# hitbc/panSVR

Hardware: AMD Instinct MI355X
Metric: signal reads realigned/sec (150 bp PE); bit-exact CIGAR vs CPU ref (higher is better)
Workload: dtype u8/int32 (2-bit k-mers, 8-bit DP deltas, 32-bit scores); 1 GPU; configs[1]: 1000000 synthetic 150 bp PE signal read pairs per GPU vs 10000-anchor SV reference (11.8 Mbp), `panSVR aln` hot path; pairs_per_gpu=1000000, engines_per_gpu=1, in_process_rebases=0, index_hbm_bytes=2713674320, index_distribution=every rank uploads its own copy from host memory

## Files before the change

pansvr_amd/csrc/aln_device.h:

```cpp
#pragma once
#include <stdint.h>
#include "../../include/psvr_engine.h"

#if defined(__HIPCC__)
#include <hip/hip_runtime.h>
#define PSVR_HD __host__ __device__ __forceinline__
#define PSVR_HDN __host__ __device__
#else
#define PSVR_HD inline
#define PSVR_HDN
#endif

namespace psvr {

static const int kLenKmer = 20, kSeedStep = 5, kUniPosNMax = 32;
static const int kMaxOut = 6;
static const int kMaxReadLen = 1600;
static const int kFwd = 1, kRev = 0;
static const int kSegMax = 160;
static const int kCigMax = 256;
static const int kMemSlot = 32;

struct SvDev { uint32_t chr_id; uint32_t st_pos; int32_t end_offset; int32_t pad; };

// ... 98 lines not shown
	DevIndex idx;
	psvr_aln_params_t par;
	int8_t mat[25];
	long long n_pairs;
	const char *bases; const long long *base_off; const psvr_ori_t *ori;
	int32_t lmax;
	int32_t wmax;
	const int32_t *grand; long long grand_n; long long grand_base;
	const int32_t *hrand[2]; long long hrand_n; long long hrand_base[2];
	long long n_slots;
	const int32_t *src;
	long long *poff;
	int32_t *rcnt;
	long long *hoff; int32_t *hcnt;
	const uint8_t *force;
	uint8_t *active; uint8_t *unmapped; uint8_t *is_str; uint8_t *has_n4;
	uint8_t *has_mem;
	int32_t *str_list; unsigned int *str_cnt;
	int32_t *read_l;
	uint8_t *bin;
	uint64_t *rb;
	uint8_t *seed_list;
	Strand *strand;
	ChainCand *ccand; int32_t *n_ccand;
	psvr_read_hdr_t *rh; psvr_pair_result_t *pres;
	psvr_cand_t *cand;
	Arena<VMem> mem; Arena<USeed> us; PathN *path;
	Arena<Seg> seg; Arena<DpDesc> dp; Arena<CandWork> cw; Arena<uint32_t> cig;
	const psvr_extz_t *dp_ez; const uint32_t *dp_cig;
	const uint8_t *tseq_in; int32_t *stale_open;
	int32_t *any_h;
	int32_t trace;
	int32_t *err;
	unsigned long long *stats;
};

enum { ST_PROBES = 0, ST_HITS, ST_SEEDS, ST_DP, ST_SIMPLE, ST_CELLS, ST_READS, ST_CAND, ST_N };

PSVR_HD void stat_add(const Ctx &c, int k, unsigned long long v)
{
	if (!c.stats) return;
#if defined(__HIP_DEVICE_COMPILE__)
	atomicAdd(c.stats + k, v);
#else
	c.stats[k] += v;
#endif
}

PSVR_HD long long src_read(const Ctx &c, long long read)
{
	return c.src ? (long long)c.src[read >> 1] * 2 + (read & 1) : read;
}

PSVR_HD uint64_t fnv1a(uint64_t h, uint64_t v)
{
	for (int i = 0; i < 8; ++i) { h ^= (v >> (8 * i)) & 0xff; h *= 1099511628211ULL; }
	return h;
}

PSVR_HD bool bucket_occupied(const DevIndex &ix, uint64_t h)
{
#ifdef PSVR_EMU_SPARSE_HASH
	(void)ix, (void)h;
	return true;
#else
	return !ix.occ || ((ix.occ[h >> 5] >> (h & 31)) & 1u);
// ... 1700 lines not shown
```

pansvr_amd/csrc/engine.hip:

```cpp
#include <hip/hip_runtime.h>
#include <algorithm>
#include <cstring>
#include <mutex>
#include <string>
#include <thread>
#include <vector>
#include "common.h"
#include "engine_core.h"
#include "bam_emit_hooks.h"
#include "fastq_parsed.h"
#include "host_io.h"
#include "index_build.h"
#include "ksw_device.h"
#include "ksw_launch.h"
#include "scan.h"

namespace psvr {

int dp_params(const psvr_ksw_params_t *par, int variant, DpParams *P);

static const int kBlock = 256;
static inline unsigned grid_for(long long n, int block = kBlock) { return (unsigned)((n + block - 1) / block); }

__device__ __forceinline__ long long pair_of(const int32_t *work, long long i) { return work ? (long long)work[i] : i; }
// ... 403 lines not shown
				if (old == km) { atomicAdd(&cnt[h], 1u); break; }
				h = (h + 1) & mask;
			}
		}
		distinct += __popcll(__ballot(fresh));
	}
	if (!((uint32_t)distinct < (uint32_t)kn - 15u)) { if (lane == 0) c.is_str[read] = 0; continue; }
	uint8_t *sl = (uint8_t *)(cnt + tsize);
	for (int i = lane; i < kn; i += 64) {
		const unsigned long long km = get_kmer((uint32_t)i, rb);
		unsigned h = (unsigned)((km * 0x9E3779B97F4A7C15ull) >> 40) & mask;
		while (key[h] != km) h = (h + 1) & mask;
		sl[i] = cnt[h] >= 4 ? 0 : 1;
	}
	if (lane == 0) {
		c.is_str[read] = 1;
		int bg = 0, ed = 0;
		for (int o = 0; o < kSeedStep; ++o) {
			bg += sl[o] == 0, ed += sl[L - kLenKmer - o] == 0;
			sl[o] += 2, sl[L - kLenKmer - o] += 4;
		}
		if (bg < kSeedStep && ed < kSeedStep) {
			int tot = 0;
			for (int o = 0; tot < kSeedStep && o < kn; ++o) {
				if (sl[o] > 0) continue;
				sl[o] += 8, tot++;
			}
		}
	}
	uint8_t *out = c.seed_list + read * (long long)c.lmax;
	for (int i = lane; i < kn; i += 64) out[i] = sl[i];
	}
}
__global__ __launch_bounds__(kBlock) __attribute__((amdgpu_waves_per_eu(8, 8))) void k_seed(Ctx c, const int32_t *work, long long n, int mate, int lds_pitch)
{
	extern __shared__ __align__(16) uint64_t seed_lds[];
	long long i = blockIdx.x * (long long)blockDim.x + threadIdx.x;
	if (i >= 2 * n) return;
	const long long rs = (pair_of(work, i >> 1) * 2 + mate) * 2 + (i & 1);
	if (lds_pitch) {
		uint64_t *mine = seed_lds + (size_t)threadIdx.x * lds_pitch;
		if (c.active[rs >> 1]) {
			const uint64_t *src = c.rb + rs * (long long)c.wmax;
			for (int k = 0; k < c.wmax; ++k) mine[k] = src[k];
		}
		seed_strand_t<true>(c, rs, mine);
	} else seed_strand_t<false>(c, rs, nullptr);
}
__global__ __launch_bounds__(kBlock) void k_scan_batch(const char *bases, const long long *off, const psvr_ori_t *ori, long long P, int match, int32_t *list, unsigned int *cnt_lmax)
{
	const long long p = blockIdx.x * (long long)blockDim.x + threadIdx.x;
	int lmax = 0, nn[2] = {0, 0};
	if (p < P) {
#pragma unroll
		for (int k = 0; k < 2; ++k) {
			const long long r = 2 * p + k, o = off[r], L = off[r + 1] - o;
			lmax = max(lmax, (int)(L < 0x7fffffff ? L : 0x7fffffff));
			const psvr_ori_t q = ori[r];
			const bool unm = q.unmapped || (uint32_t)q.chr_id > 24u;
			if ((!unm && q.align_score == (uint32_t)(L * match)) || L < kLenKmer || L > kMaxReadLen) continue;
			const uintptr_t a0 = (uintptr_t)(bases + o), a1 = a0 + (uintptr_t)L;
			int n = 0;
			for (uintptr_t a = a0 & ~(uintptr_t)3; a < a1; a += 4) {
				uint32_t x = *(const uint32_t *)a ^ 0x4E4E4E4Eu;
				if (a < a0) x |= 0xffffffffu >> (8 * (4 - (unsigned)(a0 - a)));
				if (a + 4 > a1) x |= 0xffffffffu << (8 * (unsigned)(a1 - a));
				const uint32_t z = ~(((x & 0x7F7F7F7Fu) + 0x7F7F7F7Fu) | x | 0x7F7F7F7Fu);
				n += __popc(z);
			}
			nn[k] = n < 255 ? n : 255;
		}
		if (nn[0] + nn[1] >= 1) {
// ... 14 lines not shown
	int32_t val[kListItems];
	unsigned int rank[kListItems];
	bool has[kListItems];
#pragma unroll
	for (int k = 0; k < kListItems; ++k) {
		const long long i = base + (long long)k * kBlock + threadIdx.x;
		has[k] = i < n_items && pred(i, val[k]);
		const unsigned long long m = __ballot(has[k]);
		unsigned int w0 = 0;
		if ((threadIdx.x & 63) == 0 && m) w0 = atomicAdd(&n_blk, (unsigned int)__popcll(m));
		rank[k] = (unsigned int)__builtin_amdgcn_readfirstlane((int)w0) + (unsigned int)__popcll(m & ((1ull << (threadIdx.x & 63)) - 1));
	}
	__syncthreads();
	if (threadIdx.x == 0 && n_blk) b_blk = atomicAdd(cnt, n_blk);
	__syncthreads();
#pragma unroll
	for (int k = 0; k < kListItems; ++k) if (has[k]) list[b_blk + rank[k]] = val[k];
}
__global__ __launch_bounds__(kBlock) void k_mem_list(Ctx c, const int32_t *work, long long n, int mate, int32_t *list, unsigned int *cnt)
{
	compact_list(n, list, cnt, [&](long long i, int32_t &read) {
		const long long r = pair_of(work, i) * 2 + mate;
		read = (int32_t)r;
		return c.active[r] && c.has_mem[r];
	});
}
__global__ __launch_bounds__(kBlock) void k_chain_small(Ctx c, const int32_t *list, const unsigned int *cnt)
{
	const long long i = blockIdx.x * (long long)blockDim.x + threadIdx.x;
	if (i >= (long long)*cnt) return;
	const int32_t r = list[i];
	if (chain_select_small(c, r)) return;
	chain_read(c, r), select_read(c, r);
}
__global__ __launch_bounds__(kBlock) void k_pair_dev(Ctx c, const int32_t *list, const unsigned long long *cnt)
{
	const unsigned long long n = *cnt;
	for (unsigned long long i = blockIdx.x * (unsigned long long)blockDim.x + threadIdx.x; i < n; i += (unsigned long long)gridDim.x * blockDim.x) pair_reads(c, list[i]);
}
__global__ __launch_bounds__(kBlock) void k_walk_list(Ctx c, const int32_t *work, long long n, int32_t *list, unsigned int *cnt)
{
	compact_list(2 * n, list, cnt, [&](long long i, int32_t &read) {
		const long long r = pair_of(work, i >> 1) * 2 + (i & 1);
		read = (int32_t)r;
		return c.active[r] && c.n_ccand[r] > 0;
	});
}
template <class T> __device__ __forceinline__ long long block_arena_alloc(const Arena<T> &a, unsigned long long n)
{
	__shared__ unsigned long long wsum[kBlock / 64];
	__shared__ long long bbase;
	const int lane = threadIdx.x & 63, wave = threadIdx.x >> 6, nw = (int)(blockDim.x >> 6);
	unsigned long long x = n;
#pragma unroll
	for (int o = 1; o < 64; o <<= 1) {
		const unsigned long long y = __shfl_up(x, o);
		if (lane >= o) x += y;
	}
	if (lane == 63) wsum[wave] = x;
	__syncthreads();
	if (threadIdx.x == 0) {
		unsigned long long tot = 0;
		for (int w = 0; w < nw; ++w) { const unsigned long long t = wsum[w]; wsum[w] = tot; tot += t; }
		long long b = 0;
		if (tot) {
			const unsigned long long o = atomicAdd(a.top, tot);
// ... 633 lines not shown
	}
	void unstage(Readbacks rb)
	{
		size_t at = 0;
		for (const Readback &x : rb) if (x.n) memcpy(x.h, (char *)pin + at, x.n), at += x.n;
	}
	hipEvent_t ev_early = nullptr;
	bool late_pending = false;
	int32_t *d2h_early_late(Readbacks early, const void *dl, size_t nl)
	{
		if (!ev_early && hipEventCreateWithFlags(&ev_early, hipEventDisableTiming) != hipSuccess) { d2h(early); return nullptr; }
		bool ok = true;
		const bool staged = queue_d2h(early, kLateAt, ok);
		note(hipEventRecord(ev_early, stream));
		const bool fits = staged && nl <= kPin - 4096 - kLateAt;
		if (fits) { note(hipMemcpyAsync((char *)pin + kLateAt, dl, nl, hipMemcpyDeviceToHost, stream)); late_pending = true; }
		note(hipEventSynchronize(ev_early));
		if (staged) unstage(early);
		return fits ? (int32_t *)((char *)pin + kLateAt) : nullptr;
	}
	void d2h_late_done() { if (late_pending) { note(hipStreamSynchronize(stream)); synced(); late_pending = false; } }
	~GpuBE()
	{
		if (pin) (void)hipHostFree(pin);
		if (up_ring) (void)hipHostFree(up_ring);
		if (ev_early) (void)hipEventDestroy(ev_early);
		if (ev_plan) (void)hipEventDestroy(ev_plan);
		for (int i = 0; i < kSide; ++i) {
			stream_pool().put(device, side[i]);
			if (ev_join[i]) (void)hipEventDestroy(ev_join[i]);
		}
		if (ev_fork) (void)hipEventDestroy(ev_fork);
	}
	void st_seed(const Ctx &c, const int32_t *w, long long n, int mate)
	{
		if (n > 0) {
			int pitch = c.wmax | 1;
			if ((size_t)pitch * 8 * kBlock > 64 * 1024) pitch = 0;
			t0("k_seed");
			hipLaunchKernelGGL(k_seed, dim3(grid_for(2 * n)), dim3(kBlock), (size_t)pitch * 8 * kBlock, stream, c, w, n, mate, pitch);
			t1();
			note(mem_list.ensure((size_t)(n + 4) * 4));
			note(hipMemsetAsync(mem_list.p, 0, 4, stream));
			hipLaunchKernelGGL(k_mem_list, dim3(grid_for(n, kBlock * kListItems)), dim3(kBlock), 0, stream, c, w, n, mate, mem_list.as<int32_t>() + 4, (unsigned int *)mem_list.p);
		}
		note(hipGetLastError());
	}
	DevBuf mem_list;
	void st_chain(const Ctx &c, const int32_t *w, long long n, int mate)
	{
		(void)w, (void)mate;
		if (n <= 0) return;
		t0("k_chain_small");
		hipLaunchKernelGGL(k_chain_small, dim3(grid_for(n)), dim3(kBlock), 0, stream, c, (const int32_t *)(mem_list.as<int32_t>() + 4), (const unsigned int *)mem_list.p);
		t1();
		note(hipGetLastError());
	}
	void st_pair_dev(const Ctx &c, const int32_t *list, const unsigned long long *cnt)
	{
		const long long blocks = c.n_pairs / kBlock + 1;
		hipLaunchKernelGGL(k_pair_dev, dim3((unsigned)(blocks < 2048 ? blocks : 2048)), dim3(kBlock), 0, stream, c, list, cnt);
		note(hipGetLastError());
	}
	static int str_tsize(const Ctx &c)
	{
		int tsize = 256;
		while (tsize < 2 * c.lmax) tsize <<= 1;
		return tsize;
	}
	DevBuf redo;
	static long long prep_pair_min() { static const long long v = [] { const char *e = getenv("PSVR_PREP_PAIR_MIN"); return e ? atoll(e) : 65536ll; }(); return v; }
	static int waves_for_lds(size_t per_wave, size_t fixed)
	{
		int w = kBlock / 64;
		while (w > 1 && fixed + (size_t)w * per_wave > (size_t)64 * 1024) w >>= 1;
		return w;
	}
	void launch_prep_wave(const Ctx &c, const int32_t *w, long long n, int mate, const unsigned int *n_dev, unsigned grid)
	{
		const int tsize = c.lmax <= 288 ? str_tsize(c) / 4 : str_tsize(c);
		const size_t per_wave = ((size_t)2 * c.lmax + (size_t)c.wmax * 8 + (size_t)tsize * 4 + 15) & ~(size_t)15;
		const int wpb = waves_for_lds(per_wave, 128);
		hipLaunchKernelGGL(k_prep, dim3(grid * (unsigned)(kBlock / 64 / wpb)), dim3(64 * wpb), (size_t)128 + (size_t)wpb * per_wave, stream, c, w, n, mate, tsize, (int)per_wave, n_dev);
	}
	void st_prep(const Ctx &c, const int32_t *w, long long n, int mate)
	{
		if (n <= 0) return;
		dzero(c.str_cnt, 4);
		if (c.lmax <= 288 && n >= prep_pair_min() && redo.ensure((size_t)(n + 4) * 4) == hipSuccess) {
			t0("k_prep");
			if (mate) {
				note(hipMemsetAsync(redo.p, 0, 4, stream));
				hipLaunchKernelGGL(k_prep_mate1, dim3(grid_for(n)), dim3(kBlock), 0, stream, c, w, n, redo.as<int32_t>() + 4, (unsigned int *)redo.p);
				launch_prep_wave(c, (const int32_t *)(redo.as<int32_t>() + 4), 0, 1, (const unsigned int *)redo.p, 64);
			} else if (c.lmax <= 160) hipLaunchKernelGGL((k_prep_pair<5, 256>), dim3(grid_for(n, 256)), dim3(256), (size_t)4 * 64 * (1 << (kPrepBits - 3)), stream, c, w, n, kPrepBits);
			else hipLaunchKernelGGL((k_prep_pair<9, 128>), dim3(grid_for(n, 128)), dim3(128), (size_t)2 * 64 * 512, stream, c, w, n, 12);
			t1();
			note(hipGetLastError());
			return;
		}
		t0("k_prep");
		launch_prep_wave(c, w, n, mate, nullptr, grid_for(n, kBlock / 64));
		t1();
		note(hipGetLastError());
	}
	void st_str(const Ctx &c, const int32_t *w, long long n, int mate)
	{
		if (n <= 0) return;
		const int tsize = str_tsize(c);
		const size_t per_wave = (size_t)tsize * 12 + (((size_t)c.lmax + 15) & ~(size_t)15);
		const int wpb = waves_for_lds(per_wave, 0);
		const size_t lds = (size_t)wpb * per_wave;
		t0("k_str_detect");
		const long long waves = n < 8192 ? n : 8192;
		hipLaunchKernelGGL(k_str_detect, dim3(grid_for(waves, wpb)), dim3(64 * wpb), lds, stream, c, w, n, mate, tsize, (int)per_wave);
		t1();
		note(hipGetLastError());
	}
#define PSVR_STAGE(name, kern, mult, blk)                                                                          \
	void name(const Ctx &c, const int32_t *w, long long n)                                                         \
	{                                                                                                              \
		if (n > 0) { t0(#kern); hipLaunchKernelGGL(kern, dim3(grid_for((mult) * n, blk)), dim3(blk), 0, stream, c, w, n); t1(); } \
		note(hipGetLastError());                                                                                   \
	}
	DevBuf walk_list;
	void st_walk(const Ctx &c, const int32_t *w, long long n)
	{
		if (n <= 0) return;
		note(walk_list.ensure((size_t)(2 * n + 4) * 4));
		int32_t *list = walk_list.as<int32_t>() + 4;
		unsigned int *cnt = (unsigned int *)walk_list.p;
		note(hipMemsetAsync(cnt, 0, 4, stream));
		hipLaunchKernelGGL(k_walk_list, dim3(grid_for(2 * n, kBlock * kListItems)), dim3(kBlock), 0, stream, c, w, n, list, cnt);
		t0("k_walk");
		hipLaunchKernelGGL(k_walk, dim3(grid_for(2 * n)), dim3(kBlock), 0, stream, c, (const int32_t *)list, (const unsigned int *)cnt);
		t1();
		note(hipGetLastError());
	}
	PSVR_STAGE(st_pair, k_pair, 1, kBlock)
	PSVR_STAGE(st_finalize_pair, k_finalize_pair, 1, kBlock)
#undef PSVR_STAGE
	DevBuf tmp_idx, tmp_val, tmp_out;
	void run_init(const RunInit &r)
	{
		long long n = r.S;
		for (long long k : {r.nsp, (long long)r.n_tops, (long long)r.n_atops, 16ll}) if (k > n) n = k;
		hipLaunchKernelGGL(k_run_init, dim3(grid_for(n)), dim3(kBlock), 0, stream, r);
		note(hipGetLastError());
	}
	void append_iota(int32_t *w, long long at, long long start, long long n) { if (n) hipLaunchKernelGGL(k_iota, dim3(grid_for(n)), dim3(kBlock), 0, stream, w, at, start, n); }
	void append_list(int32_t *w, long long at, const int32_t *src, long long n) { if (n) hipLaunchKernelGGL(k_copy_i32, dim3(grid_for(n)), dim3(kBlock), 0, stream, w, at, src, n); }
	void gather_listed(const long long *a, const long long *b, const int32_t *cc, const int32_t *idx, long long n, long long *oa, long long *ob, int32_t *oc)
	{
		if (!n) return;
		note(tmp_idx.ensure(n * 4)), note(tmp_out.ensure(n * 20 + 16));
		h2d(tmp_idx.p, idx, n * 4);
		hipLaunchKernelGGL(k_gather_listed, dim3(grid_for(n)), dim3(kBlock), 0, stream, a, b, cc, (const int32_t *)tmp_idx.p, n, (long long *)tmp_out.p);
		const char *o = (const char *)tmp_out.p;
		d2h({{oa, o, (size_t)n * 8}, {ob, o + n * 8, (size_t)n * 8}, {oc, o + n * 16, (size_t)n * 4}});
	}
	void scatter_listed_i32(int32_t *a, const int32_t *val, long long n)
	{
		if (!n) return;
		note(tmp_val.ensure(n * 4));
		h2d(tmp_val.p, val, n * 4);
// ... 644 lines not shown
{
	if (psvr_device_count() <= 0) return set_error(PSVR_ERR_DEVICE, "no HIP device visible: the engine has no CPU path");
	if (!e || !fq || !fq->valid || first_pair < 0 || n_pairs < 0 || first_pair + n_pairs > fq->last.n_pairs) return set_error(PSVR_ERR_ARG, "psvr_engine_upload_fastq: bad argument");
	if (fq->device != e->ix->device)
		return set_error(PSVR_ERR_ARG, "psvr_engine_upload_fastq: the text was parsed on device %d, the engine runs on device %d (the bases would have to travel between them)", fq->device, e->ix->device);
	PSVR_HIP(hipSetDevice(e->ix->device));
	e->be.stream = e->own;
	if (!e->committed) { e->core.commit(); e->committed = true; }
	e->compact_valid = false;
	e->src_fq = nullptr, e->ran = false;
	const int64_t *off = fq->base_off.as<int64_t>() + 2 * first_pair;
	long long b0 = 0, b1 = fq->last.total_bases;
	const bool whole = first_pair == 0 && n_pairs == fq->last.n_pairs;
	if (!whole && n_pairs > 0 && !e->be.d2h({{&b0, off, 8}, {&b1, off + 2 * n_pairs, 8}})) return engine_status(e, PSVR_ERR_DEVICE);
	const int rc = e->core.upload_device(n_pairs, fq->bases.as<char>(), off, fq->ori.as<psvr_ori_t>() + 2 * first_pair, b0, b1 - b0);
	const int st = engine_status(e, rc);
	if (!st) e->src_fq = fq, e->src_first = first_pair, e->src_n = n_pairs, e->src_generation = fq->generation;
	return st;
}

extern "C" int psvr_engine_run(psvr_engine_t *e, int trace, void *stream)
{
	if (!e) return set_error(PSVR_ERR_ARG, "psvr_engine_run: null engine");
	PSVR_HIP(hipSetDevice(e->ix->device));
	e->be.stream = stream ? (hipStream_t)stream : e->own;
	e->be.timing = (trace & 4) != 0;
	e->be.timed.clear();
	e->compact_valid = false;
	int rc = e->core.run(trace & 1, (trace & 2) != 0);
	hipError_t s = hipStreamSynchronize(e->be.stream);
	if (s != hipSuccess) e->be.note(s);
	e->be.synced();
	e->be.collect_timing();
	e->committed = false;
	const int st = engine_status(e, rc);
	e->ran = st == PSVR_OK;
	return st;
}

extern "C" int psvr_engine_set_stream_pos(psvr_engine_t *e, const int64_t pos[3])
{
	if (!e || !pos) return set_error(PSVR_ERR_ARG, "psvr_engine_set_stream_pos: null argument");
	PSVR_HIP(hipSetDevice(e->ix->device));
	e->core.have_run = false, e->committed = true;
	e->core.grand_pos = pos[0], e->core.hrand_pos[0] = pos[1], e->core.hrand_pos[1] = pos[2];
	return PSVR_OK;
}

extern "C" int psvr_engine_stream_end(psvr_engine_t *e, int64_t end[3])
{
	if (!e || !end) return set_error(PSVR_ERR_ARG, "psvr_engine_stream_end: null argument");
	PSVR_HIP(hipSetDevice(e->ix->device));
	long long t[3];
	e->core.stream_end(t);
	end[0] = t[0], end[1] = t[1], end[2] = t[2];
	return engine_status(e, PSVR_OK);
}

extern "C" int psvr_engine_rebase(psvr_engine_t *e, const int64_t pos[3], void *stream)
{
	if (!e || !pos) return set_error(PSVR_ERR_ARG, "psvr_engine_rebase: null argument");
	PSVR_HIP(hipSetDevice(e->ix->device));
	e->be.stream = stream ? (hipStream_t)stream : e->own;
	e->compact_valid = false;
	int rc = e->core.rebase(pos[0], pos[1], pos[2], e->core.c.trace, false);
	hipError_t s = hipStreamSynchronize(e->be.stream);
// ... 76 lines not shown
{
	std::lock_guard<std::mutex> lk(ix->emit_mu);
	if (!ix->emit_ready) {
		int cur = -1;
		(void)hipGetDevice(&cur);
		struct Back { int d; ~Back() { if (d >= 0) (void)hipSetDevice(d); } } back{cur};
		PSVR_HIP(hipSetDevice(ix->device));
		BeTableHost h;
		h.build((int)ix->host.svh.size(), [&](int i) { return ix->host.svh[(size_t)i].vcf_print_string.c_str(); }, [&](int i) { return ix->host.svh[(size_t)i].vcf_id.c_str(); });
		PSVR_HIP(ix->emit_text.alloc(h.text.size())); PSVR_HIP(ix->emit_off.alloc(h.off.size() * 4)); PSVR_HIP(ix->emit_tab.alloc(h.tab.size()));
		PSVR_HIP(hipMemcpy(ix->emit_text.p, h.text.data(), h.text.size(), hipMemcpyHostToDevice));
		PSVR_HIP(hipMemcpy(ix->emit_off.p, h.off.data(), h.off.size() * 4, hipMemcpyHostToDevice));
		PSVR_HIP(hipMemcpy(ix->emit_tab.p, h.tab.data(), h.tab.size(), hipMemcpyHostToDevice));
		ix->emit_ready = true;
	}
	T->text = ix->emit_text.as<char>(), T->off = ix->emit_off.as<uint32_t>(), T->tab = ix->emit_tab.as<uint8_t>();
	T->n_anchor = (int32_t)ix->host.svh.size(), T->n_header = ix->host.n_header;
	*device = ix->device;
	return PSVR_OK;
}
void psvr::engine_emit_view(const psvr_engine *e, EngineEmitView *v)
{
	const Ctx &c = e->core.c;
	v->device = e->ix->device, v->ran = e->ran && e->core.P > 0;
	v->fq = e->src_fq, v->first_pair = e->src_first, v->n_pairs = e->src_n, v->generation = e->src_generation;
	v->hdr = c.rh, v->pairs = c.pres, v->cands = c.cand, v->n_cands = (int64_t)c.cw.cap, v->cig = c.cig.base, v->n_cig = (int64_t)c.cig.cap;
}

extern "C" int psvr_engine_stats(const psvr_engine_t *e, char *buf, size_t n)
{
	if (!e || !buf || !n) return set_error(PSVR_ERR_ARG, "psvr_engine_stats: bad argument");
	const RunStats &s = e->core.stats;
	snprintf(buf, n,
	         "{\"pairs\":%lld,\"rounds\":%lld,\"pair_runs\":%lld,\"pair_only_runs\":%lld,\"shadow_runs\":%lld,\"sensitive_pairs\":%lld,\"window_misses\":%lld,\"adopted_pairs\":%lld,\"stale_open\":%lld,\"dp_problems\":%lld,\"dp_seq_bytes\":%lld,\"candidates\":%lld,\"walk_pairs\":%lld,\"walk_us\":%lld,\"n_special\":%lld,\"special_const\":%lld,\"special_nomove\":%lld,"
	         "\"probes\":%llu,\"hits\":%llu,\"seeds\":%llu,\"dp_cells\":%llu,\"simple\":%llu,\"reads_aligned\":%llu}",
	         e->core.P, s.rounds, s.pairs_run, s.pair_only, s.shadow_runs, s.sensitive, s.window_miss, s.adopted, s.stale_open, s.dp_problems, s.dp_seq_bytes, s.cands, s.walk_pairs, s.walk_us, s.n_special, s.special_const, s.special_nomove, s.counters[ST_PROBES], s.counters[ST_HITS], s.counters[ST_SEEDS],
	         s.counters[ST_CELLS], s.counters[ST_SIMPLE], s.counters[ST_READS]);
	std::string t = buf;
	t.pop_back();
	{
		size_t fr = 0, tot = 0;
		char b[96];
		if (hipSetDevice(e->ix->device) == hipSuccess && hipMemGetInfo(&fr, &tot) == hipSuccess) { snprintf(b, sizeof b, ",\"hbm_used_bytes\":%zu", tot - fr); t += b; }
	}
	t += ",\"kernels\":{";
	bool first = true;
	for (auto &k : e->be.timed) {
		char b[256];
		snprintf(b, sizeof b, "%s\"%s\":{\"ms\":%.4f,\"launches\":%lld}", first ? "" : ",", k.first.c_str(), k.second.first, k.second.second);
		t += b, first = false;
	}
	t += "}}";
	snprintf(buf, n, "%s", t.c_str());
	return PSVR_OK;
}
```

pansvr_amd/csrc/engine_core.h:

```cpp
#pragma once
#include <stdint.h>
#include <stdio.h>
#include <string.h>
#include <algorithm>
#include <atomic>
#include <cstdlib>
#include <initializer_list>
#include <mutex>
#include <string>
#include <thread>
#include <chrono>
#include <type_traits>
#include <vector>
#include "aln_device.h"
#include "dp_plan.h"

namespace psvr {

struct HostRand3 {
	int32_t ring[31];
	int f, b;
	void seed(unsigned s)
	{
		int32_t word = s ? (int32_t)s : 1;
// ... 41 lines not shown
		want = (want + 0xfffff) & ~0xfffffll;
		for (; k < want; ++k) {
			int32_t *&b = blk[k >> kLog];
			if (!b) b = new int32_t[(size_t)1 << kLog];
			b[k & kMask] = gen.next();
		}
		n.store(k, std::memory_order_release);
	}
	int32_t at(long long k) const { return blk[k >> kLog][k & kMask]; }
	void prefetch(long long k) const { if (k >= 0 && k < n.load(std::memory_order_relaxed)) __builtin_prefetch(blk[k >> kLog] + (k & kMask)); }
	template <class F> void pieces(long long from, long long cnt, F &&put) const
	{
		for (long long o = 0; o < cnt;) {
			const long long k = from + o, room = (kMask + 1) - (k & kMask), m = cnt - o < room ? cnt - o : room;
			put(o, blk[k >> kLog] + (k & kMask), m);
			o += m;
		}
	}
};
inline SharedRand &shared_grand() { static SharedRand s; return s; }

struct DpIO {
	long long begin, end;
	int32_t *qlen, *tlen;
	long long *q_off, *t_off;
	uint8_t *qbuf, *tbuf;
	psvr_extz_t *ez;
	uint32_t *cig;
	long long qbytes, tbytes, cig_words;
};

template <class B, class = void> struct plans_on_device : std::false_type {};
template <class B> struct plans_on_device<B, std::void_t<decltype(B::kDevicePlan)>> : std::true_type {};

struct Readback { void *h; const void *d; size_t n; };
typedef std::initializer_list<Readback> Readbacks;

struct HostMem {
	struct Buf {
		void *p = nullptr;
		size_t bytes = 0;
		Buf() = default;
		Buf(const Buf &) = delete;
		Buf &operator=(const Buf &) = delete;
		~Buf() { release(); }
		void release() { free(p); p = nullptr; bytes = 0; }
		bool alloc(size_t n)
		{
			release();
			p = calloc(n ? n : 1, 1);
			bytes = p ? n : 0;
			return p != nullptr;
		}
	};
	bool note(bool ok) { return ok; }
	void d2h(Readbacks rb) { for (const Readback &x : rb) if (x.n) memcpy(x.h, x.d, x.n); }
	void d2h(void *h, const void *d, size_t n) { d2h({{h, d, n}}); }
	std::vector<int32_t> late_buf;
	int32_t *d2h_early_late(Readbacks early, const void *dl, size_t nl)
	{
		d2h(early);
		late_buf.resize(nl / 4 + 1);
		memcpy(late_buf.data(), dl, nl);
		return late_buf.data();
	}
	void d2h_late_done() {}
	std::vector<int32_t> listed_idx;
	void gather_listed(const long long *a, const long long *b, const int32_t *cc, const int32_t *idx, long long n, long long *oa, long long *ob, int32_t *oc)
	{
		if (!n) return;
		listed_idx.assign(idx, idx + n);
		for (long long i = 0; i < n; ++i) oa[i] = a[idx[i]], ob[i] = b[idx[i]], oc[i] = cc[idx[i]];
	}
	void scatter_listed_i32(int32_t *a, const int32_t *val, long long n) { for (long long i = 0; i < n; ++i) a[listed_idx[i]] = val[i]; }
};

struct RunStats {
	long long rounds = 0, pairs_run = 0, pair_only = 0, shadow_runs = 0, sensitive = 0, window_miss = 0, dp_problems = 0, cands = 0, adopted = 0, stale_open = 0, dp_seq_bytes = 0, from_walk = 0;
	long long walk_pairs = 0, walk_us = 0, n_special = 0, special_const = 0, special_nomove = 0;
	unsigned long long counters[16] = {0};
};

template <class BE, class Mem = HostMem> struct EngineCore {
	BE &be;
	HostMem host;
	Mem &mem;
	typedef typename Mem::Buf Buf;
	template <class T> struct Dev : Buf { operator T *() const { return (T *)this->p; } };
	bool alloc_ok = true;
	template <class T> T *get(Dev<T> &b, unsigned long long n) { alloc_ok &= mem.note(b.alloc((n ? n : 1) * sizeof(T))); return b; }
	Ctx c;
	long long P = 0, R = 0;
	long long total_bases = 0;
	SharedRand &grand = shared_grand();
	RandStream hrand[2];
	long long grand_pos = 0, hrand_pos[2] = {0, 0};
	long long grand_dev_n = 0, hrand_dev_n = 0;
	long long grand_dev_base = 0, hrand_dev_base[2] = {0, 0}, grand_dev_cap = 0, hrand_dev_cap = 0;
	Dev<int32_t> d_grand, d_hrand[2];
	struct {
		Dev<long long> poff, hoff;
		Dev<int32_t> rcnt, hcnt, str_list, read_l, n_ccand;
		Dev<unsigned int> str_cnt;
		Dev<uint8_t> active, unmapped, is_str, has_n4, has_mem, bin, seed_list;
		Dev<uint64_t> rb;
		Dev<Strand> strand;
		Dev<ChainCand> ccand;
		Dev<psvr_read_hdr_t> rh;
		Dev<psvr_pair_result_t> pres;
		Dev<unsigned long long> stats;
		Dev<VMem> mem;
// ... 177 lines not shown
		c.rb = get(cb.rb, (unsigned long long)RS * 2 * c.wmax);
		c.seed_list = get(cb.seed_list, (unsigned long long)RS * c.lmax);
		c.strand = get(cb.strand, 2 * RS);
		c.ccand = get(cb.ccand, 12 * RS), c.n_ccand = get(cb.n_ccand, RS);
		c.rh = get(cb.rh, RS), c.pres = get(cb.pres, S);
		get(d_work, S), get(d_workp, P);
		get(d_ctot, S), get(d_src, S), get(d_sens, P), get(d_slist, P);
		get(d_hprev, 2 * S);
		get(d_force, 8 * S), get(d_mask, P), get(d_cmask, P);
		get(d_hasn, P), get(d_resel, P), get(d_resel4, P < kReselCap ? P : kReselCap);
		{
			const long long nsp = S / 4 + 1;
			get(d_vsrc, S), get(d_spidx, nsp);
			get(d_special, nsp), get(d_sp_class, nsp), get(d_sp_adopted, nsp), get(d_sp_adopted_at, nsp);
		}
		get(d_tops, 64), get(d_atops, 6 * kTopStride), get(d_flags, 16);
		const long long R2 = RS;
		cap_mem = (unsigned long long)2 * R2 * kMemSlot + (unsigned long long)R2 * 16 + 4096;
		cap_us = (unsigned long long)R2 * 48 + 65536;
		cap_cw = (unsigned long long)R2 * 3 + 1024;
		cap_seg = cap_cw * 16;
		cap_dp = (unsigned long long)R2 * 4 + 1024;
		cap_cig = (unsigned long long)R2 * 48 + 4096;
		if (const char *e = getenv("PSVR_ARENA_SHRINK")) {
			const unsigned long long n = (unsigned long long)atoll(e);
			if (n > 1) {
				for (unsigned long long *cap : {&cap_us, &cap_cw, &cap_seg, &cap_dp, &cap_cig}) *cap = *cap / n + 64;
				const unsigned long long slots = (unsigned long long)2 * R2 * kMemSlot;
				cap_mem = slots + (cap_mem - slots) / n + 64;
			}
		}
		c.stats = get(cb.stats, 16);
		if (!alloc_ok || !alloc_arenas()) { cap_S = 0; err = "device allocation failed"; return PSVR_ERR_NOMEM; }
		c.err = d_flags + 6, c.stale_open = d_flags + 7, c.any_h = d_flags + 8;
		upload_variants();
		return PSVR_OK;
	}

	void upload_variants()
	{
		{
			std::vector<uint8_t> force((size_t)8 * V, 0);
			h_vsrc.assign(V, 0), h_sp_idx.assign(special.size(), 0);
			for (size_t i = 0; i < special.size(); ++i) {
				const Special &sp = special[i];
				h_sp_idx[i] = sp.pair;
				for (int v = 0; v < sp.nvar; ++v) {
					long long slot = sp.vslot + v;
					h_vsrc[slot - P] = sp.pair;
					int code = v;
					for (int k = 0; k < 2; ++k) {
						int n = k == 0 ? sp.n1 : sp.n2;
						uint8_t *f = &force[4 * (2 * (slot - P) + k)];
						f[0] = (uint8_t)n;
						for (int j = 0; j < n; ++j) f[1 + j] = (uint8_t)(code & 3), code >>= 2;
					}
				}
			}
			be.dzero(d_force, (size_t)8 * S);
			if (V) be.h2d(d_force + (size_t)8 * P, force.data(), force.size());
			be.dzero(d_hasn, (size_t)P);
			if (!special.empty()) {
				be.h2d(d_special, special.data(), special.size() * sizeof(Special));
				be.h2d(d_spidx, h_sp_idx.data(), h_sp_idx.size() * 4);
			}
			if (V) be.h2d(d_vsrc, h_vsrc.data(), V * 4);
			if (!h_n_idx.empty()) be.scatter_u8(d_hasn, h_n_idx.data(), (long long)h_n_idx.size(), 1);
// ... 14 lines not shown
		return alloc_ok;
	}
	int grow_and_rerun(const int32_t *flags, int trace, bool want_stats, int depth)
	{
		if (depth > 8) { err = "scratch arena overflow persists after 8 growth steps"; return PSVR_ERR_OVERFLOW; }
		unsigned long long *caps[6] = {&cap_mem, &cap_us, &cap_seg, &cap_dp, &cap_cw, &cap_cig};
		for (int k = 0; k < 6; ++k) if (flags[k]) *caps[k] *= 4;
		if (flags[0]) cap_mem += (unsigned long long)4 * S * kMemSlot;
		fprintf(stderr, "[psvr] scratch arena overflow (mem %d us %d seg %d dp %d cand %d cigar %d): growing 4x and re-running the batch\n", flags[0], flags[1], flags[2], flags[3],
		        flags[4], flags[5]);
		if (!alloc_arenas()) { cap_S = 0; err = "device allocation failed while growing arenas"; return PSVR_ERR_NOMEM; }
		return run(trace, want_stats, depth + 1);
	}

	bool ensure_dp(long long n, long long qb, long long tb, long long cw)
	{
		auto room = [](long long need) { return need + need / 4 + 1024; };
		alloc_ok = true;
		if (n + 2 > dp_cap_n) {
			dp_cap_n = room(n + 2);
			dp.qlen = get(dpb.qlen, dp_cap_n), dp.tlen = get(dpb.tlen, dp_cap_n), dp.q_off = get(dpb.q_off, dp_cap_n), dp.t_off = get(dpb.t_off, dp_cap_n);
			dp.ez = get(dpb.ez, dp_cap_n);
		}
		if (qb + 64 > dp_cap_q) dp.qbuf = get(dpb.qbuf, dp_cap_q = room(qb + 64));
		if (tb + 64 > dp_cap_t) dp.tbuf = get(dpb.tbuf, dp_cap_t = room(tb + 64));
		if (cw + 64 > dp_cap_c) dp.cig = get(dpb.cig, dp_cap_c = room(cw + 64));
		if (!alloc_ok) dp_cap_n = dp_cap_q = dp_cap_t = dp_cap_c = 0;
		return alloc_ok;
	}

	int run_slots(const int32_t *work, long long nwork, long long &dp_done, long long &cw_done, long long nwalk = 0)
	{
		if (nwork + nwalk <= 0) return PSVR_OK;
		for (int mate = 0; mate < 2; ++mate) {
			be.st_prep(c, work, nwork, mate);
			be.st_str(c, work, nwork, mate);
			be.st_seed(c, work, nwork, mate);
			be.st_chain(c, work, nwork, mate);
		}
		be.st_walk(c, work, nwork + nwalk);
		int32_t fl[16];
		long long dp_end, cw_end;
		if constexpr (plans_on_device<BE>::value) {
			int rc = be.st_dp_plan(*this, dp_done, dp_end, cw_end, fl);
			if (rc) return rc;
		} else {
			unsigned long long tops[kTopStride + 1];
			mem.d2h({{tops, d_atops + 3 * kTopStride, sizeof tops}, {fl, d_flags, 64}});
			dp_end = (long long)tops[0], cw_end = (long long)tops[kTopStride];
		}
		if (fl[8]) any_h = true;
		if (fl[7]) stats.stale_open = 1;
		{
			const int full = (dp_end > (long long)cap_dp || fl[3] ? 1 : 0) | (cw_end > (long long)cap_cw || fl[4] ? 2 : 0) | (fl[2] ? 4 : 0) | (fl[1] ? 8 : 0) | (fl[0] ? 16 : 0);
			if (full) return -1000 - full;
		}
		if (dp_end > dp_done) {
			dp.begin = dp_done, dp.end = dp_end;
			int rc = be.st_dp(*this);
			if (rc) return rc;
		}
		c.dp_ez = dp.ez ? dp.ez - dp_done : nullptr, c.dp_cig = dp.cig;
		if (cw_end > cw_done) be.st_assemble(c, cw_done, cw_end);
		stats.dp_problems += dp_end - dp_done, stats.cands += cw_end - cw_done;
		dp_done = dp_end, cw_done = cw_end;
		be.st_finalize_pair(c, work, nwork + nwalk);
		return PSVR_OK;
	}

	struct Win { int32_t pair; long long eval_off; int32_t eval_tot; std::vector<long long> off; std::vector<int32_t> tot; };
	std::vector<int32_t> w_listed, w_cur_tot, w_res;
	std::vector<long long> w_pre, w_cur_off;
	std::vector<int32_t> h_vsrc, h_sp_idx;
	struct HostTable {
		int32_t *p = nullptr;
		size_t n = 0, cap = 0;
		bool empty() const { return n == 0; }
		void clear() { n = 0; }
		int32_t *data() { return p; }
		const int32_t &operator[](size_t i) const { return p[i]; }
		bool resize(size_t want)
		{
			if (want > cap) {
				free(p);
				cap = want + want / 4 + 1024;
// ... 344 lines not shown
```

Before: 375.0 million reads/s.

## Seed both mates in one launch and re-seed only mismatched mate-1 reads

Result: faster. 379.2 million reads/s, median of 6 (+1.1%).

```diff
diff --git a/pansvr_amd/csrc/aln_device.h b/pansvr_amd/csrc/aln_device.h
--- a/pansvr_amd/csrc/aln_device.h
+++ b/pansvr_amd/csrc/aln_device.h
@@ -154,6 +154,7 @@
 	int32_t *any_h;
 	int32_t trace;
 	int32_t *err;
+	int32_t *late_n;
 	unsigned long long *stats;
 };
 
diff --git a/pansvr_amd/csrc/engine.hip b/pansvr_amd/csrc/engine.hip
--- a/pansvr_amd/csrc/engine.hip
+++ b/pansvr_amd/csrc/engine.hip
@@ -459,12 +459,13 @@
 	for (int i = lane; i < kn; i += 64) out[i] = sl[i];
 	}
 }
+template <int MATES>
 __global__ __launch_bounds__(kBlock) __attribute__((amdgpu_waves_per_eu(8, 8))) void k_seed(Ctx c, const int32_t *work, long long n, int mate, int lds_pitch)
 {
 	extern __shared__ __align__(16) uint64_t seed_lds[];
 	long long i = blockIdx.x * (long long)blockDim.x + threadIdx.x;
-	if (i >= 2 * n) return;
-	const long long rs = (pair_of(work, i >> 1) * 2 + mate) * 2 + (i & 1);
+	if (i >= 2 * MATES * n) return;
+	const long long rs = MATES == 2 ? pair_of(work, i >> 2) * 4 + (i & 3) : (pair_of(work, i >> 1) * 2 + mate) * 2 + (i & 1);
 	if (lds_pitch) {
 		uint64_t *mine = seed_lds + (size_t)threadIdx.x * lds_pitch;
 		if (c.active[rs >> 1]) {
@@ -545,6 +546,41 @@
 	const int32_t r = list[i];
 	if (chain_select_small(c, r)) return;
 	chain_read(c, r), select_read(c, r);
+}
+enum { LC_MEM0 = 0, LC_MEM1, LC_LATE, LC_WALK, LC_N };
+__global__ __launch_bounds__(kBlock) void k_mem_list_mate1(Ctx c, const int32_t *work, long long n, int32_t *list, unsigned int *cnt, int32_t *late)
+{
+	if (blockIdx.x == 0 && threadIdx.x == 0) *c.str_cnt = 0;
+	compact_list(n, list, cnt + LC_MEM1, [&](long long i, int32_t &read) {
+		const long long slot = pair_of(work, i), r = slot * 2 + 1;
+		read = (int32_t)r;
+		const int32_t v = c.rcnt[slot * 3 + 1];
+		if (v & kPrepMark) {
+			c.rcnt[slot * 3 + 1] = v & 0x3ff;
+			if (c.rcnt[slot * 3] != ((v >> 10) & 0x3ff)) {
+				if (c.stats) atomicAdd(c.stats + ST_READS, ~0ull);
+				late[atomicAdd(cnt + LC_LATE, 1u)] = (int32_t)slot;
+				return false;
+			}
+		}
+		return c.active[r] && c.has_mem[r];
+	});
+}
+__global__ __launch_bounds__(kBlock) void k_seed_late(Ctx c, const int32_t *late, const unsigned int *cnt)
+{
+	const long long n = 2 * (long long)cnt[LC_LATE];
+	for (long long i = blockIdx.x * (long long)blockDim.x + threadIdx.x; i < n; i += (long long)gridDim.x * blockDim.x)
+		seed_strand_t<false>(c, ((long long)late[i >> 1] * 2 + 1) * 2 + (i & 1), nullptr);
+}
+__global__ __launch_bounds__(kBlock) void k_chain_late(Ctx c, const int32_t *late, const unsigned int *cnt)
+{
+	const long long n = (long long)cnt[LC_LATE];
+	if (blockIdx.x == 0 && threadIdx.x == 0 && n) atomicAdd(c.late_n, (int32_t)n);
+	for (long long i = blockIdx.x * (long long)blockDim.x + threadIdx.x; i < n; i += (long long)gridDim.x * blockDim.x) {
+		const long long r = (long long)late[i] * 2 + 1;
+		if (!c.active[r] || !c.has_mem[r]) continue;
+		if (!chain_select_small(c, r)) chain_read(c, r), select_read(c, r);
+	}
 }
 __global__ __launch_bounds__(kBlock) void k_pair_dev(Ctx c, const int32_t *list, const unsigned long long *cnt)
 {
@@ -1244,28 +1280,81 @@
 		}
 		if (ev_fork) (void)hipEventDestroy(ev_fork);
 	}
+	static int seed_pitch(const Ctx &c)
+	{
+		const int pitch = c.wmax | 1;
+		return (size_t)pitch * 8 * kBlock > 64 * 1024 ? 0 : pitch;
+	}
+	DevBuf mem_list, list_cnt;
+	unsigned int *lc(int k) { return (unsigned int *)list_cnt.p + k; }
+	bool lc_zeroed = false;
 	void st_seed(const Ctx &c, const int32_t *w, long long n, int mate)
 	{
 		if (n > 0) {
-			int pitch = c.wmax | 1;
-			if ((size_t)pitch * 8 * kBlock > 64 * 1024) pitch = 0;
+			const int pitch = seed_pitch(c);
 			t0("k_seed");
-			hipLaunchKernelGGL(k_seed, dim3(grid_for(2 * n)), dim3(kBlock), (size_t)pitch * 8 * kBlock, stream, c, w, n, mate, pitch);
+			hipLaunchKernelGGL(k_seed<1>, dim3(grid_for(2 * n)), dim3(kBlock), (size_t)pitch * 8 * kBlock, stream, c, w, n, mate, pitch);
 			t1();
-			note(mem_list.ensure((size_t)(n + 4) * 4));
-			note(hipMemsetAsync(mem_list.p, 0, 4, stream));
-			hipLaunchKernelGGL(k_mem_list, dim3(grid_for(n, kBlock * kListItems)), dim3(kBlock), 0, stream, c, w, n, mate, mem_list.as<int32_t>() + 4, (unsigned int *)mem_list.p);
+			note(mem_list.ensure((size_t)(2 * n + 8) * 4)), note(list_cnt.ensure(64));
+			note(hipMemsetAsync(lc(LC_MEM0), 0, 4, stream));
+			hipLaunchKernelGGL(k_mem_list, dim3(grid_for(n, kBlock * kListItems)), dim3(kBlock), 0, stream, c, w, n, mate, mem_list.as<int32_t>(), lc(LC_MEM0));
 		}
 		note(hipGetLastError());
 	}
-	DevBuf mem_list;
 	void st_chain(const Ctx &c, const int32_t *w, long long n, int mate)
 	{
 		(void)w, (void)mate;
 		if (n <= 0) return;
 		t0("k_chain_small");
-		hipLaunchKernelGGL(k_chain_small, dim3(grid_for(n)), dim3(kBlock), 0, stream, c, (const int32_t *)(mem_list.as<int32_t>() + 4), (const unsigned int *)mem_list.p);
+		hipLaunchKernelGGL(k_chain_small, dim3(grid_for(n)), dim3(kBlock), 0, stream, c, (const int32_t *)mem_list.as<int32_t>(), (const unsigned int *)lc(LC_MEM0));
 		t1();
+		note(hipGetLastError());
+	}
+	static constexpr bool kPairRound = true;
+	bool pair_round(const Ctx &c, long long n)
+	{
+		return c.lmax <= 288 && n >= prep_pair_min() && redo.ensure((size_t)(n + 4) * 4) == hipSuccess && mem_list.ensure((size_t)(2 * n + 8) * 4) == hipSuccess && list_cnt.ensure(64) == hipSuccess;
+	}
+	void st_seed_both(const Ctx &c, const int32_t *w, long long n)
+	{
+		const int pitch = seed_pitch(c);
+		t0("k_seed");
+		hipLaunchKernelGGL(k_seed<2>, dim3(grid_for(4 * n)), dim3(kBlock), (size_t)pitch * 8 * kBlock, stream, c, w, n, 0, pitch);
+		t1();
+		note(hipMemsetAsync(list_cnt.p, 0, 4 * LC_N, stream));
+		lc_zeroed = true;
+		hipLaunchKernelGGL(k_mem_list, dim3(grid_for(n, kBlock * kListItems)), dim3(kBlock), 0, stream, c, w, n, 0, mem_list.as<int32_t>(), lc(LC_MEM0));
+		note(hipGetLastError());
+	}
+	void st_chain_mate1(const Ctx &c, const int32_t *w, long long n)
+	{
+		int32_t *late = redo.as<int32_t>(), *list1 = mem_list.as<int32_t>() + n;
+		hipLaunchKernelGGL(k_mem_list_mate1, dim3(grid_for(n, kBlock * kListItems)), dim3(kBlock), 0, stream, c, w, n, list1, lc(0), late);
+		const bool fork = !timing && side_streams();
+		hipStream_t launch = stream;
+		if (fork) {
+			note(hipEventRecord(ev_fork, launch));
+			note(hipStreamWaitEvent(side[1], ev_fork, 0));
+			stream = side[1];
+		}
+		t0("k_prep");
+		launch_prep_wave(c, late, 0, 1, lc(LC_LATE), 64);
+		t1();
+		st_str(c, w, n, 1);
+		t0("k_seed");
+		hipLaunchKernelGGL(k_seed_late, dim3(64), dim3(kBlock), 0, stream, c, (const int32_t *)late, (const unsigned int *)lc(0));
+		t1();
+		t0("k_chain_small");
+		hipLaunchKernelGGL(k_chain_late, dim3(64), dim3(kBlock), 0, stream, c, (const int32_t *)late, (const unsigned int *)lc(0));
+		t1();
+		if (fork) {
+			note(hipEventRecord(ev_join[1], side[1]));
+			stream = launch;
+		}
+		t0("k_chain_small");
+		hipLaunchKernelGGL(k_chain_small, dim3(grid_for(n)), dim3(kBlock), 0, stream, c, (const int32_t *)list1, (const unsigned int *)lc(LC_MEM1));
+		t1();
+		if (fork) note(hipStreamWaitEvent(stream, ev_join[1], 0));
 		note(hipGetLastError());
 	}
 	void st_pair_dev(const Ctx &c, const int32_t *list, const unsigned long long *cnt)
@@ -1299,12 +1388,12 @@
 	{
 		if (n <= 0) return;
 		dzero(c.str_cnt, 4);
-		if (c.lmax <= 288 && n >= prep_pair_min() && redo.ensure((size_t)(n + 4) * 4) == hipSuccess) {
+		if (c.lmax <= 288 && n >= prep_pair_min() && redo.ensure((size_t)(n + 4) * 4) == hipSuccess && list_cnt.ensure(64) == hipSuccess) {
 			t0("k_prep");
 			if (mate) {
-				note(hipMemsetAsync(redo.p, 0, 4, stream));
-				hipLaunchKernelGGL(k_prep_mate1, dim3(grid_for(n)), dim3(kBlock), 0, stream, c, w, n, redo.as<int32_t>() + 4, (unsigned int *)redo.p);
-				launch_prep_wave(c, (const int32_t *)(redo.as<int32_t>() + 4), 0, 1, (const unsigned int *)redo.p, 64);
+				note(hipMemsetAsync(lc(LC_LATE), 0, 4, stream));
+				hipLaunchKernelGGL(k_prep_mate1, dim3(grid_for(n)), dim3(kBlock), 0, stream, c, w, n, redo.as<int32_t>(), lc(LC_LATE));
+				launch_prep_wave(c, (const int32_t *)redo.as<int32_t>(), 0, 1, lc(LC_LATE), 64);
 			} else if (c.lmax <= 160) hipLaunchKernelGGL((k_prep_pair<5, 256>), dim3(grid_for(n, 256)), dim3(256), (size_t)4 * 64 * (1 << (kPrepBits - 3)), stream, c, w, n, kPrepBits);
 			else hipLaunchKernelGGL((k_prep_pair<9, 128>), dim3(grid_for(n, 128)), dim3(128), (size_t)2 * 64 * 512, stream, c, w, n, 12);
 			t1();
@@ -1339,10 +1428,11 @@
 	void st_walk(const Ctx &c, const int32_t *w, long long n)
 	{
 		if (n <= 0) return;
-		note(walk_list.ensure((size_t)(2 * n + 4) * 4));
-		int32_t *list = walk_list.as<int32_t>() + 4;
-		unsigned int *cnt = (unsigned int *)walk_list.p;
-		note(hipMemsetAsync(cnt, 0, 4, stream));
+		note(walk_list.ensure((size_t)(2 * n + 4) * 4)), note(list_cnt.ensure(64));
+		int32_t *list = walk_list.as<int32_t>();
+		unsigned int *cnt = lc(LC_WALK);
+		if (!lc_zeroed) note(hipMemsetAsync(cnt, 0, 4, stream));
+		lc_zeroed = false;
 		hipLaunchKernelGGL(k_walk_list, dim3(grid_for(2 * n, kBlock * kListItems)), dim3(kBlock), 0, stream, c, w, n, list, cnt);
 		t0("k_walk");
 		hipLaunchKernelGGL(k_walk, dim3(grid_for(2 * n)), dim3(kBlock), 0, stream, c, (const int32_t *)list, (const unsigned int *)cnt);
@@ -2053,6 +2143,7 @@
 	if (s != hipSuccess) e->be.note(s);
 	e->be.synced();
 	e->be.collect_timing();
+	if (trace & 1) fprintf(stderr, "[psvr] batch of %lld pairs: %lld rounds, %lld of them seeded both mates in one go, %lld mate-1 reads seeded again\n", e->core.P, e->core.stats.rounds, e->core.stats.paired_rounds, e->core.stats.late_mate1);
 	e->committed = false;
 	const int st = engine_status(e, rc);
 	e->ran = st == PSVR_OK;
@@ -2195,9 +2286,9 @@
 	if (!e || !buf || !n) return set_error(PSVR_ERR_ARG, "psvr_engine_stats: bad argument");
 	const RunStats &s = e->core.stats;
 	snprintf(buf, n,
-	         "{\"pairs\":%lld,\"rounds\":%lld,\"pair_runs\":%lld,\"pair_only_runs\":%lld,\"shadow_runs\":%lld,\"sensitive_pairs\":%lld,\"window_misses\":%lld,\"adopted_pairs\":%lld,\"stale_open\":%lld,\"dp_problems\":%lld,\"dp_seq_bytes\":%lld,\"candidates\":%lld,\"walk_pairs\":%lld,\"walk_us\":%lld,\"n_special\":%lld,\"special_const\":%lld,\"special_nomove\":%lld,"
+	         "{\"pairs\":%lld,\"rounds\":%lld,\"pair_runs\":%lld,\"pair_only_runs\":%lld,\"shadow_runs\":%lld,\"sensitive_pairs\":%lld,\"window_misses\":%lld,\"adopted_pairs\":%lld,\"stale_open\":%lld,\"dp_problems\":%lld,\"dp_seq_bytes\":%lld,\"candidates\":%lld,\"walk_pairs\":%lld,\"walk_us\":%lld,\"n_special\":%lld,\"special_const\":%lld,\"special_nomove\":%lld,\"paired_rounds\":%lld,\"late_mate1\":%lld,"
 	         "\"probes\":%llu,\"hits\":%llu,\"seeds\":%llu,\"dp_cells\":%llu,\"simple\":%llu,\"reads_aligned\":%llu}",
-	         e->core.P, s.rounds, s.pairs_run, s.pair_only, s.shadow_runs, s.sensitive, s.window_miss, s.adopted, s.stale_open, s.dp_problems, s.dp_seq_bytes, s.cands, s.walk_pairs, s.walk_us, s.n_special, s.special_const, s.special_nomove, s.counters[ST_PROBES], s.counters[ST_HITS], s.counters[ST_SEEDS],
+	         e->core.P, s.rounds, s.pairs_run, s.pair_only, s.shadow_runs, s.sensitive, s.window_miss, s.adopted, s.stale_open, s.dp_problems, s.dp_seq_bytes, s.cands, s.walk_pairs, s.walk_us, s.n_special, s.special_const, s.special_nomove, s.paired_rounds, s.late_mate1, s.counters[ST_PROBES], s.counters[ST_HITS], s.counters[ST_SEEDS],
 	         s.counters[ST_CELLS], s.counters[ST_SIMPLE], s.counters[ST_READS]);
 	std::string t = buf;
 	t.pop_back();
diff --git a/pansvr_amd/csrc/engine_core.h b/pansvr_amd/csrc/engine_core.h
--- a/pansvr_amd/csrc/engine_core.h
+++ b/pansvr_amd/csrc/engine_core.h
@@ -97,6 +97,8 @@
 
 template <class B, class = void> struct plans_on_device : std::false_type {};
 template <class B> struct plans_on_device<B, std::void_t<decltype(B::kDevicePlan)>> : std::true_type {};
+template <class B, class = void> struct seeds_both_mates : std::false_type {};
+template <class B> struct seeds_both_mates<B, std::void_t<decltype(B::kPairRound)>> : std::true_type {};
 
 struct Readback { void *h; const void *d; size_t n; };
 typedef std::initializer_list<Readback> Readbacks;
@@ -142,6 +144,7 @@
 
 struct RunStats {
 	long long rounds = 0, pairs_run = 0, pair_only = 0, shadow_runs = 0, sensitive = 0, window_miss = 0, dp_problems = 0, cands = 0, adopted = 0, stale_open = 0, dp_seq_bytes = 0, from_walk = 0;
+	long long paired_rounds = 0, late_mate1 = 0;
 	long long walk_pairs = 0, walk_us = 0, n_special = 0, special_const = 0, special_nomove = 0;
 	unsigned long long counters[16] = {0};
 };
@@ -385,7 +388,7 @@
 		}
 		c.stats = get(cb.stats, 16);
 		if (!alloc_ok || !alloc_arenas()) { cap_S = 0; err = "device allocation failed"; return PSVR_ERR_NOMEM; }
-		c.err = d_flags + 6, c.stale_open = d_flags + 7, c.any_h = d_flags + 8;
+		c.err = d_flags + 6, c.stale_open = d_flags + 7, c.any_h = d_flags + 8, c.late_n = d_flags + 9;
 		upload_variants();
 		return PSVR_OK;
 	}
@@ -466,7 +469,16 @@
 	int run_slots(const int32_t *work, long long nwork, long long &dp_done, long long &cw_done, long long nwalk = 0)
 	{
 		if (nwork + nwalk <= 0) return PSVR_OK;
-		for (int mate = 0; mate < 2; ++mate) {
+		bool paired = false;
+		if constexpr (seeds_both_mates<BE>::value) if (be.pair_round(c, nwork)) {
+			be.st_prep(c, work, nwork, 0);
+			be.st_str(c, work, nwork, 0);
+			be.st_seed_both(c, work, nwork);
+			be.st_chain(c, work, nwork, 0);
+			be.st_chain_mate1(c, work, nwork);
+			stats.paired_rounds++, paired = true;
+		}
+		if (!paired) for (int mate = 0; mate < 2; ++mate) {
 			be.st_prep(c, work, nwork, mate);
 			be.st_str(c, work, nwork, mate);
 			be.st_seed(c, work, nwork, mate);
@@ -485,6 +497,7 @@
 		}
 		if (fl[8]) any_h = true;
 		if (fl[7]) stats.stale_open = 1;
+		stats.late_mate1 = fl[9];
 		{
 			const int full = (dp_end > (long long)cap_dp || fl[3] ? 1 : 0) | (cw_end > (long long)cap_cw || fl[4] ? 2 : 0) | (fl[2] ? 4 : 0) | (fl[1] ? 8 : 0) | (fl[0] ? 16 : 0);
 			if (full) return -1000 - full;
```
